# frgfm/Holocron

Hardware: AMD Instinct MI355X
Metric: images/sec fwd+bwd+AdaBelief, RepVGG-A0 bs256/GPU 224^2 (higher is better)
Workload: dtype bf16; 1 GPU; repvgg_a0 bf16 train step (fwd+bwd+AdaBelief), synthetic 224^2, bs=256 per MI355X (BASELINE.json configs[1]), random-init weights, 10 classes, CE label_smoothing 0.1; global_batch=256, parallelism=dp1, mode=weight gradients on a second stream; hipGraph replay of the full step, dump_outputs=/tmp/code/gt15__hip_graft__frgfm__Holocron/driver_out/dump_parent, deterministic=True

## Files before the change

### holocron_amd/_lib.py

```python
import ctypes as C
import os

import torch

_HERE = os.path.dirname(os.path.abspath(__file__))
LIB_PATH = os.environ.get("HC_LIB_PATH") or os.path.join(_HERE, "lib", "libholocron_hip.so")

HC_MAX_TAPS = 12
HC_MT_CHUNK = 8192
HC_STAT_REPLICAS = 128

c_void_p, c_int32, c_int64, c_float, c_double = C.c_void_p, C.c_int32, C.c_int64, C.c_float, C.c_double


class ConvClass(C.Structure):
    _fields_ = [("OHg", c_int32), ("OWg", c_int32), ("oy0", c_int32), ("ox0", c_int32), ("ostep", c_int32),
                ("istep", c_int32), ("ntaps", c_int32), ("tap", c_int32 * HC_MAX_TAPS)]


class ConvDesc(C.Structure):
    _fields_ = [("src0", c_void_p), ("src1", c_void_p), ("wpk", c_void_p), ("dst", c_void_p), ("resid", c_void_p),
                ("stats", c_void_p), ("bias", c_void_p), ("act", c_int32),
                ("N", c_int32), ("IH", c_int32), ("IW", c_int32), ("srcC", c_int32),
                ("OH", c_int32), ("OW", c_int32), ("Cout", c_int32), ("T", c_int32), ("nclass", c_int32),
# ... 162 lines not shown
    "hc_yolo1_loss_fwd": (c_int32, [c_void_p] * 3 + [c_int32] * 8 + [c_void_p] * 4 + [c_int32] + [c_void_p] * 4),
    "hc_yolo1_loss_bwd": (c_int32, [c_void_p] * 3 + [c_int32] * 8 + [c_void_p] * 4 + [c_int32] + [c_void_p] * 7),
    "hc_yolo1_decode": (c_int32, [c_void_p] * 3 + [c_int32] * 7 + [c_void_p] * 4),
    "hc_yolo_format_fwd": (c_int32, [c_void_p] * 2 + [c_int32] * 7 + [c_void_p] * 5),
    "hc_yolo_format_bwd": (c_int32, [c_void_p] * 3 + [c_int32] * 7 + [c_void_p] * 7),
    "hc_lamb_step": (c_int32, [c_void_p, c_int32, c_void_p, c_void_p, c_void_p, c_int32, c_void_p]),
    "hc_tadam_step": (c_int32, [c_void_p, c_int32, c_void_p, c_void_p, c_void_p, c_void_p, c_void_p, c_void_p, c_int32, c_void_p]),
    "hc_adan_step": (c_int32, [c_void_p, c_void_p, c_int32, c_void_p, c_void_p]),
    "hc_lookahead_sync": (c_int32, [c_void_p, c_int32, c_float, c_void_p]),
    "hc_multi_copy": (c_int32, [C.POINTER(MultiCopyDesc), c_void_p]),
    "hc_msbn_finalize": (c_int32, [C.POINTER(MsbnDesc), c_void_p]),
    "hc_msbn_bwd_finalize": (c_int32, [C.POINTER(MsbnDesc), c_void_p]),
    "hc_msbn_apply": (c_int32, [C.POINTER(MsbnIo), c_void_p, c_void_p, c_void_p, c_int32, c_void_p]),
    "hc_msbn_bwd_reduce": (c_int32, [C.POINTER(MsbnIo), c_void_p, c_int32, c_void_p, c_void_p, c_int32, c_void_p]),
    "hc_msbn_bwd_apply": (c_int32, [C.POINTER(MsbnIo), c_void_p, c_int32, c_void_p, c_void_p, c_int32, c_void_p]),
    "hc_dwrep_dgrad": (c_int32, [c_void_p, c_void_p, c_int32, c_void_p, c_void_p] + [c_int32] * 5 + [c_void_p]),
    "hc_conv_gather": (c_int32, [C.POINTER(ConvDesc), c_void_p]),
    "hc_conv_pointwise_supported": (c_int32, [C.POINTER(ConvDesc)]),
    "hc_conv_pointwise": (c_int32, [C.POINTER(ConvDesc), c_void_p]),
    "hc_conv_small": (c_int32, [C.POINTER(ConvSmallDesc), c_void_p]),
    "hc_conv_small_supported": (c_int32, [C.POINTER(ConvSmallDesc)]),
    "hc_conv_rows_fused_bwd_supported": (c_int32, [C.POINTER(ConvSmallDesc)]),
    "hc_conv_rows_fused_bwd": (c_int32, [C.POINTER(ConvSmallDesc), c_void_p, c_void_p, c_int32] + [c_void_p] * 8),
    "hc_conv_s2_supported": (c_int32, [C.POINTER(ConvS2Desc)]),
    "hc_conv_s2_fwd": (c_int32, [C.POINTER(ConvS2Desc), c_void_p]),
    "hc_conv_s2_dgrad_supported": (c_int32, [C.POINTER(ConvS2DgradDesc)]),
    "hc_conv_s2_dgrad": (c_int32, [C.POINTER(ConvS2DgradDesc), c_void_p]),
    "hc_conv_s2_stem_wgrad_ws_bytes": (c_int64, []),
    "hc_conv_s2_stem_wgrad": (c_int32, [c_void_p] * 6 + [c_int32] * 4 + [c_void_p]),
    "hc_conv_wgrad_ws_bytes": (c_int64, [C.POINTER(WgradDesc)]),
    "hc_conv_wgrad": (c_int32, [C.POINTER(WgradDesc), c_void_p]),
    "hc_conv_wgrad_group_supported": (c_int32, [C.POINTER(WgradGroupDesc)]),
    "hc_conv_wgrad_group_ws_bytes": (c_int64, [C.POINTER(WgradGroupDesc)]),
    "hc_conv_wgrad_group": (c_int32, [C.POINTER(WgradGroupDesc), c_void_p]),
    "hc_rep_wgrad_supported": (c_int32, [C.POINTER(RepWgradDesc)]),
    "hc_rep_wgrad_ws_bytes": (c_int64, [C.POINTER(RepWgradDesc)]),
    "hc_rep_wgrad_plan": (c_int32, [C.POINTER(RepWgradDesc), c_void_p]),
    "hc_rep_wgrad": (c_int32, [C.POINTER(RepWgradDesc), c_void_p]),
    "hc_pack_conv_weight": (c_int32, [c_void_p, c_void_p] + [c_int32] * 7 + [c_void_p]),
    "hc_pack_conv_weights_multi": (c_int32, [c_void_p, c_int32, c_int64, c_void_p]),
    "hc_nchw_to_nhwc_bf16": (c_int32, [c_void_p, c_void_p] + [c_int32] * 5 + [c_void_p]),
    "hc_nhwc_bf16_to_nchw": (c_int32, [c_void_p, c_void_p] + [c_int32] * 5 + [c_void_p]),
    "hc_im2col_small": (c_int32, [c_void_p, c_void_p] + [c_int32] * 11 + [c_void_p]),
    "hc_unpack_im2col_grad": (c_int32, [c_void_p, c_void_p] + [c_int32] * 6 + [c_void_p]),
    "hc_rep_bn_finalize": (c_int32, [C.POINTER(RepBnDesc), c_void_p]),
    "hc_rep_apply": (c_int32, [c_void_p] * 6 + [c_int64, c_int32, c_int32, c_void_p]),
# ... 152 lines not shown
```

### holocron_amd/csrc/conv_rows48.hip

```cpp
#include <type_traits>
#include "common.h"
#include "../../include/holocron_hip.h"

namespace crq {

constexpr int NT = 512, C = 48, CK = 2, PSC = C / 8 + 1, PS = PSC * 16, S3 = 9 * CK, S1 = CK, S = S3 + S1;
static_assert((PS / 8) % 4 == 2, "pixel pitch must be 2 x odd 8-byte units");

struct Args {
    hc_conv_small_desc d;
    int reps;
    int nunits;
    int delay;
};

template <int W>
struct Geo {
    static constexpr int RW = W > 64 ? 1 : 2;
    static constexpr int SEGW = (W + 15) / 16;
    static constexpr int NF = RW * SEGW;
    static constexpr int UR = 4 * RW;
    static constexpr int WW = W + 1;
    static constexpr int NSLOT = (UR + 2) * WW + 1;
    static constexpr int NDMA = (NSLOT * PS + 1023) / 1024;
    static constexpr int WIN = NDMA * 1024;
    static constexpr int SMEM = 2 * WIN + 64 + 1024;
    static_assert(SMEM <= 160 * 1024, "LDS budget");
};

__device__ __forceinline__ u32x4 uniform_rsrc(const void* p, unsigned bytes) {
    const unsigned long long v = reinterpret_cast<unsigned long long>(p);
    u32x4 r;
    r[0] = __builtin_amdgcn_readfirstlane((unsigned)v);
    r[1] = __builtin_amdgcn_readfirstlane((unsigned)(v >> 32) & 0xffffu);
    r[2] = __builtin_amdgcn_readfirstlane(bytes);
    r[3] = 0x00020000u;
    return r;
}
__device__ __forceinline__ bf16x8 frag2(const char* lo_p, const char* hi_p) {
    const u32x2 lo = *reinterpret_cast<const u32x2*>(lo_p), hi = *reinterpret_cast<const u32x2*>(hi_p);
    const u32x4 v = {lo[0], lo[1], hi[0], hi[1]};
    return __builtin_bit_cast(bf16x8, v);
}
__device__ __forceinline__ float row16_sum(float v) {
    v += __builtin_bit_cast(float, __builtin_amdgcn_update_dpp(0, __builtin_bit_cast(int, v), 0x128, 0xf, 0xf, false));
    v += __builtin_bit_cast(float, __builtin_amdgcn_update_dpp(0, __builtin_bit_cast(int, v), 0x124, 0xf, 0xf, false));
    v += __builtin_bit_cast(float, __builtin_amdgcn_update_dpp(0, __builtin_bit_cast(int, v), 0x122, 0xf, 0xf, false));
    v += __builtin_bit_cast(float, __builtin_amdgcn_update_dpp(0, __builtin_bit_cast(int, v), 0x121, 0xf, 0xf, false));
    return v;
}

template <int W, int MODE, int DBG>
__global__ __launch_bounds__(NT, 1) void conv_rows48_kernel(const Args a) {
    using G = Geo<W>;
    constexpr int WW = G::WW, NF = G::NF, UR = G::UR, RW = G::RW, SEGW = G::SEGW;
    extern __shared__ __attribute__((aligned(1024))) char smem[];
    const hc_conv_small_desc& d = a.d;
    const int tid = threadIdx.x, lane = tid & 63;
    const int wid = __builtin_amdgcn_readfirstlane(tid >> 6);
    const int team = wid >> 2, pw = wid & 3;
    const int H = d.H, UPI = H / UR;
    const unsigned lds0 = hc_lds_addr(smem);
    const int px = lane & 15, g = lane >> 4;
    const int region = team * G::WIN;
    int* cnt = reinterpret_cast<int*>(smem + 2 * G::WIN) + team * 8;
    int gen = 0;

    if (tid < 16) reinterpret_cast<int*>(smem + 2 * G::WIN)[tid] = 0;
    __syncthreads();

    auto team_sync = [&]() __attribute__((always_inline)) {
        asm volatile("s_waitcnt vmcnt(0) lgkmcnt(0)" ::: "memory");
        gen += 4;
        if (lane == 0) __hip_atomic_fetch_add(cnt, 1, __ATOMIC_RELAXED, __HIP_MEMORY_SCOPE_WORKGROUP);
        while (__hip_atomic_load(cnt, __ATOMIC_RELAXED, __HIP_MEMORY_SCOPE_WORKGROUP) < gen) __builtin_amdgcn_s_sleep(1);
        asm volatile("" ::: "memory");
    };

    const unsigned act_bytes = (unsigned)d.N * H * W * C * 2u;
    const u32x4 rsA = uniform_rsrc(d.srcA, act_bytes);
    const u32x4 rsB = uniform_rsrc(MODE == 1 ? d.srcB : d.srcA, act_bytes);
    const __amdgpu_buffer_rsrc_t rsw = make_rsrc(d.w3, (unsigned)(S * C * 64));

    const unsigned wl = (unsigned)((lane & 15) * 64 + g * 16);
    u32x4 af[3][3];
    auto load_a = [&](int buf, int s) __attribute__((always_inline)) {
        if (DBG & 4) return;
#pragma unroll
        for (int f = 0; f < 3; ++f) af[buf][f] = buf_load16(rsw, wl, (unsigned)(s * (C * 64) + f * 1024));
    };

    auto stage_window = [&](const u32x4 rs, int n, int row0, int j0, int j1) __attribute__((always_inline)) {
        if (DBG & 8) return;
        const unsigned img = (unsigned)n * (unsigned)(H * W * C * 2);
        for (int j = j0 + pw; j < j1; j += 4) {
            const int J = j * 64 + lane;
            const int slot = J / PSC, c = J - slot * PSC;
            const int r = slot / WW, x = slot - r * WW;
            const int ih = row0 - 1 + r;
            const bool ok = c < PSC - 1 && slot < G::NSLOT && x >= 1 && ih >= 0 && ih < H;
            const unsigned off = img + (unsigned)((ih * W + x - 1) * C * 2 + c * 16);
            hc_dma16(rs, lds0 + (unsigned)(region + j * 1024), ok ? off : HC_OOB);
        }
    };

    const int vb = region + ((pw * RW + 1) * WW + px + 1) * PS + g * 8;
    bf16x8 bfr[2][NF];
    auto load_b = [&](int buf, int bofs, int second) __attribute__((always_inline)) {
        if (DBG & 2) return;
        const char* sb = smem + vb + bofs;
#pragma unroll
        for (int i = 0; i < NF; ++i) {
            const int o = ((i / SEGW) * WW + 16 * (i % SEGW)) * PS;
            bfr[buf][i] = frag2(sb + o, sb + o + second);
        }
    };

    f32x4 acc[3][NF];
    auto zero_acc = [&]() __attribute__((always_inline)) {
#pragma unroll
        for (int f = 0; f < 3; ++f)
#pragma unroll
            for (int i = 0; i < NF; ++i) acc[f][i] = f32x4{0.f, 0.f, 0.f, 0.f};
    };
    auto mfma_step = [&](int ab, int bb) __attribute__((always_inline)) {
#pragma unroll
        for (int i = 0; i < NF; ++i)
#pragma unroll
            for (int f = 0; f < 3; ++f) {
                if (DBG & 1) acc[f][i][0] += __builtin_bit_cast(float, af[ab][f][0]) * (float)bfr[bb][i][0];
                else acc[f][i] = __builtin_amdgcn_mfma_f32_16x16x32_bf16(__builtin_bit_cast(bf16x8, af[ab][f]), bfr[bb][i], acc[f][i], 0, 0, 0);
            }
    };
    auto step = [&](int a3, int par, int s, int bnext, int second_next, bool prefetch) __attribute__((always_inline)) {
        if (s + 2 < S) load_a((a3 + 2) % 3, s + 2);
        if (prefetch) load_b(par ^ 1, bnext, second_next);
        __builtin_amdgcn_sched_barrier(0);
        mfma_step(a3, par);
        __builtin_amdgcn_sched_barrier(0);
    };

    const int cbase = 8 * g;
    auto epilogue = [&](void* outp, float* stats, const void* residp, int n, int row0) __attribute__((always_inline)) {
        if (DBG & 16) {
            float t = 0.f;
#pragma unroll
            for (int f = 0; f < 3; ++f)
#pragma unroll
                for (int i = 0; i < NF; ++i) t += acc[f][i][0];
            if (t == 123.456f) reinterpret_cast<float*>(outp)[tid] = t;
            return;
        }
        const size_t img = (size_t)n * H * W * C;
        __builtin_amdgcn_sched_barrier(0);
        float st[2][12];
#pragma unroll
        for (int k = 0; k < 2; ++k)
#pragma unroll
            for (int e = 0; e < 12; ++e) st[k][e] = 0.f;
#pragma unroll
        for (int i = 0; i < NF; ++i) {
            const int row = row0 + pw * RW + i / SEGW, col = 16 * (i % SEGW) + px;
            const bool ok = col < W;
            const size_t e0 = img + (size_t)(row * W + (ok ? col : 0)) * C + cbase;
            bf16_t* op = reinterpret_cast<bf16_t*>(outp) + e0;
            const bf16_t* rp = residp != nullptr ? reinterpret_cast<const bf16_t*>(residp) + e0 : nullptr;
            u32x4 r16 = {0u, 0u, 0u, 0u};
            u32x2 r8 = {0u, 0u};
            if (rp != nullptr && ok) {
                r16 = *reinterpret_cast<const u32x4*>(rp);
                r8 = *reinterpret_cast<const u32x2*>(rp + 32 - 4 * g);
            }
            u32x2 pk[3];
#pragma unroll
            for (int f = 0; f < 3; ++f) {
                f32x4 v = acc[f][i];
                if (stats != nullptr) {
#pragma unroll
                    for (int e = 0; e < 4; ++e) {
                        const float x = ok ? v[e] : 0.f;
                        st[0][f * 4 + e] += x;
                        st[1][f * 4 + e] += x * x;
                    }
                }
                const unsigned ra = f == 0 ? r16[0] : (f == 1 ? r16[2] : r8[0]), rb = f == 0 ? r16[1] : (f == 1 ? r16[3] : r8[1]);
                v[0] += bf16lo(ra); v[1] += bf16hi(ra); v[2] += bf16lo(rb); v[3] += bf16hi(rb);
                pk[f] = u32x2{pack_bf16x2(v[0], v[1]), pack_bf16x2(v[2], v[3])};
            }
            if (ok) {
                *reinterpret_cast<u32x4*>(op) = u32x4{pk[0][0], pk[0][1], pk[1][0], pk[1][1]};
                *reinterpret_cast<u32x2*>(op + 32 - 4 * g) = pk[2];
            }
        }
        if (stats != nullptr) {
            float* rep = stats + (size_t)((blockIdx.x * 8 + wid) % a.reps) * 2 * C + cbase;
#pragma unroll
            for (int k = 0; k < 2; ++k) {
                float mine = 0.f;
#pragma unroll
                for (int e = 0; e < 12; ++e) {
                    const float x = row16_sum(st[k][e]);
                    mine = px == e ? x : mine;
                }
                if (px < 12) atomicAdd(rep + k * C + (px < 8 ? px : 24 - 4 * g + px), mine);
            }
        }
    };

    if (team == 1)
        for (int i = 0; i < a.delay; ++i) __builtin_amdgcn_s_sleep(64);
    bool first = true;
    for (int u = 2 * blockIdx.x + team; u < a.nunits; u += 2 * gridDim.x) {
        const int n = u / UPI, row0 = (u - n * UPI) * UR;
        if (!first) team_sync();
        first = false;
        stage_window(rsA, n, row0, 0, G::NDMA);
        load_a(0, 0);
        load_a(1, 1);
        team_sync();
        zero_acc();
        load_b(0, (-WW - 1) * PS, 32);
#pragma nounroll
        for (int kh = 0; kh < 3; ++kh) {
            const int rofs = (kh - 1) * WW * PS;
#pragma unroll
            for (int t = 0; t < 6; ++t) {
                const int kw = t >> 1, kk = t & 1;
                int bnext, second;
                bool pf = true;
                if (kk == 0) { bnext = rofs + (kw - 1) * PS + 64; second = 0; }
                else if (t < 5) { bnext = rofs + kw * PS; second = 32; }
                else {
                    bnext = kh < 2 ? kh * WW * PS - PS : 0;
                    second = 32;
                    pf = kh < 2 || MODE == 0;
                }
                step(t % 3, kk, 6 * kh + t, bnext, second, pf);
            }
        }
        if (MODE == 0) {
            epilogue(d.out3, d.stats3, nullptr, n, row0);
            zero_acc();
        } else {
            team_sync();
            stage_window(rsB, n, row0, (WW * PS) / 1024, ((UR + 1) * WW * PS + PS + 1023) / 1024);
            team_sync();
            load_b(0, 0, 32);
        }
        step(0, 0, S3, 64, 0, true);
        step(1, 1, S3 + 1, 0, 0, false);
        if (MODE == 0) epilogue(d.out1, d.stats1, nullptr, n, row0);
        else epilogue(d.out3, nullptr, d.resid, n, row0);
    }
}

template <int W>
bool shape_ok(const hc_conv_small_desc& d) {
    return d.C == C && d.Cout == C && d.W == W && d.H >= Geo<W>::UR && d.H % Geo<W>::UR == 0 && d.N >= 1 &&
           (double)d.N * d.H * d.W * C * 2.0 < 2147483000.0;
}

template <int W, int MODE, int DBG>
void launch1(const Args& a, hipStream_t st) {
    auto kern = conv_rows48_kernel<W, MODE, DBG>;
    constexpr int smem = Geo<W>::SMEM;
    static bool attr_set = false;
    if (!attr_set) {
        (void)hipFuncSetAttribute(reinterpret_cast<const void*>(kern), hipFuncAttributeMaxDynamicSharedMemorySize, smem);
        attr_set = true;
    }
    int grid = (a.nunits + 1) / 2;
    if (grid > 256) grid = 256;
    hipLaunchKernelGGL(kern, dim3(grid), dim3(NT), smem, st, a);
}

template <int W>
void launch(Args& a, hipStream_t st) {
    static const int dbg = getenv("HC_CRQ_DBG") ? atoi(getenv("HC_CRQ_DBG")) : 0;
    constexpr int delay = 2;
    a.nunits = a.d.N * (a.d.H / Geo<W>::UR);
    a.delay = delay;
    const bool dg = (a.d.mode & 1) == 1;
#define CRQ_CASE(k) case k: if (dg) launch1<W, 1, k>(a, st); else launch1<W, 0, k>(a, st); break;
    switch (dbg) {
        CRQ_CASE(1) CRQ_CASE(2) CRQ_CASE(4) CRQ_CASE(7) CRQ_CASE(8) CRQ_CASE(16) CRQ_CASE(24) CRQ_CASE(31)
        default: if (dg) launch1<W, 1, 0>(a, st); else launch1<W, 0, 0>(a, st); break;
    }
#undef CRQ_CASE
}

}

bool hc_conv_rows48_supported(const hc_conv_small_desc& d) {
    static const int on = [] { const char* e = getenv("HC_CONV_ROWS48"); return e == nullptr ? 1 : atoi(e); }();
    if (on <= 0 || (d.mode & HC_CONV_SMALL_ROWS_IMAGE) == 0 || (d.mode & ~(HC_CONV_SMALL_ROWS_IMAGE | 1)) != 0) return false;
    if ((d.mode & 1) && on < 2) return false;
    return crq::shape_ok<112>(d) || crq::shape_ok<56>(d);
}
int hc_conv_rows48_launch(const hc_conv_small_desc& d, hipStream_t st) {
    if (!hc_conv_rows48_supported(d)) return HC_ERR_ARG;
    const bool dg = (d.mode & 1) == 1;
    if (d.srcA == nullptr || d.w3 == nullptr || d.out3 == nullptr) return HC_ERR_ARG;
    if (!dg && d.out1 == nullptr) return HC_ERR_ARG;
    if (dg && d.srcB == nullptr) return HC_ERR_ARG;
    if (!dg && (d.stats3 == nullptr) != (d.stats1 == nullptr)) return HC_ERR_ARG;
    crq::Args a;
    a.d = d;
    a.reps = hc_get_stat_replicas();
    if (d.W == 112) crq::launch<112>(a, st);
    else crq::launch<56>(a, st);
    return hc_launch_status();
}
```

### holocron_amd/nn/repblock_op.py

```python
import ctypes as C

import os

import torch

from .. import _lib
from .._lib import ConvS2Desc, ConvS2DgradDesc, PackItem, RepBnBwdDesc, RepBnDesc, StemBwdDesc, StemDesc, check, ptr, stream
from ..ops import conv as cv

STEM_KPAD = 32
FUSED_BWD = os.environ.get("HC_REP_FUSED_BWD", "1") != "0"


class ZeroPool:

    def __init__(self):
        self.buf = None
        self.used = 0
        self.high = 0
        self.depth = 0
        self.gen = 0
        self.retired = []
        self.graph_users = 0
        self.buf_captured = False

    def _retire(self):
        if self.buf is not None and self.buf_captured:
            self.retired.append(self.buf)
        self.buf, self.buf_captured = None, False

    def release_retired(self):
        self.graph_users = max(0, self.graph_users - 1)
        if self.graph_users == 0:
            self.retired = []
# ... 85 lines not shown
class RepState:

    def __init__(self, stride, identity):
        self.stride = stride
        self.identity = identity
        self.emit_stats = False
        self.fwd_cache = cv.PackCache()
        self.bwd_cache = cv.PackCache()
        self.desc = {}
        self.bn = None
        self.eps = 1e-5
        self.momentum = 0.1
        self.training = True
        self.last_out_stats = None
        self.packed = None
        self.packed_key = None
        self.pack_table = {}
        self.rows_image = (False, False)
        self.stack_fwd = False
        self.s2 = False
        self.s2_images = None
        self.s2_dgrad = False
        self.s2_dimg = None

    @staticmethod
    def weights_key(w3, w1):
        return (w3.data_ptr(), w3._version, w1.data_ptr(), w1._version, cv.weights_epoch())

    def pack_items(self, w3, w1):
        Cout, Cin = w3.shape[0], w3.shape[1]
        dev = w3.device
        stem = (Cin % 16) != 0
        if self.s2:
            return self._pack_items_s2(w3, w1, Cout, Cin, dev, stem)
        self.stack_fwd = (stem or (self.stride == 2 and Cin <= 48)) and Cout % 4 == 0
        if self.packed is None or self.packed[0].device != dev:
            if self.stack_fwd:
                self.packed = (torch.zeros((2 * Cout, 1, STEM_KPAD) if stem else (2 * Cout, 9, Cin), dtype=torch.bfloat16, device=dev),
                               None, None if stem else torch.empty((Cin, 10, Cout), dtype=torch.bfloat16, device=dev))
            elif any(self.rows_image):
                rf, rb = self.rows_image
                self.packed = (cv.rows_image(Cout, dev) if rf else torch.empty((Cout, 9, Cin), dtype=torch.bfloat16, device=dev),
                               None if rf else torch.empty((Cout, 1, Cin), dtype=torch.bfloat16, device=dev),
                               cv.rows_image(Cout, dev) if rb else torch.empty((Cin, 10, Cout), dtype=torch.bfloat16, device=dev))
            elif stem:
                self.packed = (torch.zeros((Cout, 1, STEM_KPAD), dtype=torch.bfloat16, device=dev),
                               torch.zeros((Cout, 1, STEM_KPAD), dtype=torch.bfloat16, device=dev), None)
            else:
                self.packed = (torch.empty((Cout, 9, Cin), dtype=torch.bfloat16, device=dev),
                               torch.empty((Cout, 1, Cin), dtype=torch.bfloat16, device=dev),
                               torch.empty((Cin, 10, Cout), dtype=torch.bfloat16, device=dev))
            self.packed_key = None
        wp3, wp1, wpd = self.packed
        if self.stack_fwd:
            if stem:
                return [(w3, wp3, Cout, Cin, 3, 3, 2, 0, STEM_KPAD), (w1, wp3[Cout:], Cout, Cin, 1, 1, 2, 4 * Cin, STEM_KPAD)]
            return [(w3, wp3, Cout, Cin, 3, 3, 0, 0, 9), (w1, wp3[Cout:], Cout, Cin, 1, 1, 0, 4, 9),
                    (w3, wpd, Cout, Cin, 3, 3, 1, 0, 10), (w1, wpd, Cout, Cin, 1, 1, 1, 9, 10)]
        if any(self.rows_image):
            rf, rb = self.rows_image
            fwd = ([(w3, wp3, Cout, Cin, 3, 3, 3, 0, 10), (w1, wp3, Cout, Cin, 1, 1, 3, 9, 10)] if rf else
                   [(w3, wp3, Cout, Cin, 3, 3, 0, 0, 9), (w1, wp1, Cout, Cin, 1, 1, 0, 0, 1)])
            bwd = ([(w3, wpd, Cout, Cin, 3, 3, 4, 0, 10), (w1, wpd, Cout, Cin, 1, 1, 4, 9, 10)] if rb else
                   [(w3, wpd, Cout, Cin, 3, 3, 1, 0, 10), (w1, wpd, Cout, Cin, 1, 1, 1, 9, 10)])
            return fwd + bwd
        if stem:
            return [(w3, wp3, Cout, Cin, 3, 3, 2, 0, STEM_KPAD), (w1, wp1, Cout, Cin, 1, 1, 2, 4 * Cin, STEM_KPAD)]
        return [(w3, wp3, Cout, Cin, 3, 3, 0, 0, 9), (w1, wp1, Cout, Cin, 1, 1, 0, 0, 1),
                (w3, wpd, Cout, Cin, 3, 3, 1, 0, 10), (w1, wpd, Cout, Cin, 1, 1, 1, 9, 10)]

    def _pack_items_s2(self, w3, w1, Cout, Cin, dev, stem):
        if stem:
            s3, s1, s1b, mode, tap1 = 2, 1, 0, 6, 4
        else:
            pt = Cin // 8
# ... 53 lines not shown
                dg = None
            sf = sd = None
            rows = (False, False)
            if Cin % 16 == 0 and s == 1:
                sf = cv.conv_small_desc(N, H, W, Cin, Cout, cv.ROWS_IMAGE)
                sd = cv.conv_small_desc(N, H, W, Cout, Cin, cv.ROWS_IMAGE | 1)
                rows = (sf is not None, sd is not None)
                if sf is None:
                    sf = cv.conv_small_desc(N, H, W, Cin, Cout, 0)
                if sd is None:
                    sd = cv.conv_small_desc(N, H, W, Cout, Cin, 1)
            s2d = None
            if s == 2:
                c = ConvS2Desc()
                c.N, c.H, c.W, c.Cin, c.Cout, c.x_nchw_f32 = N, H, W, Cin, Cout, 1 if Cin % 16 else 0
                if _lib.load().hc_conv_s2_supported(C.byref(c)):
                    s2d = c
            s2g = None
            if s == 2 and s2d is not None and Cin % 16 == 0:
                c = ConvS2DgradDesc()
                c.N, c.H, c.W, c.Cin, c.Cout = N, H, W, Cin, Cout
                if _lib.load().hc_conv_s2_dgrad_supported(C.byref(c)):
                    s2g = c
            self.desc[key] = (f3, f1, dg, sf, sd, rows, s2d, s2g)
        rows = self.desc[key][5]
        s2, s2g = self.desc[key][6] is not None, self.desc[key][7] is not None
        if rows != self.rows_image or s2 != self.s2 or s2g != self.s2_dgrad:
            self.rows_image, self.s2, self.s2_dgrad, self.packed, self.packed_key = rows, s2, s2g, None, None
        return self.desc[key][:5]

    def s2_desc(self, N, Cin, H, W, Cout):
        self.descs(N, Cin, H, W, Cout)
        return self.desc[(N, Cin, H, W, Cout)][6]


def _stats_of(x):
    st = getattr(x, "_hc_stats", None)
    if st is not None:
        return st
    N, Cc, H, W = x.shape
    st = POOL.take((_lib.stat_replicas(), 2, Cc), x.device)
    with cv.profiled("bn_elementwise", 0.0, N * H * W * Cc * 2.0):
        check(_lib.load().hc_channel_stats(ptr(x), ptr(st), N * H * W, Cc, stream()), "hc_channel_stats")
    return st


def block_convs_forward(st, src, w3, w1, geom, stats=None, stem_cin=None):
    N, Cin, H, W, Cout = geom
    f3, f1, _, sf, _ = st.descs(N, Cin, H, W, Cout)
    OH, OW = f3.OH, f3.OW
    dev = src.device
# ... 47 lines not shown
        cv.launch_conv_small_dgrad(sdg, dy3, dy1, wpd, dx, resid=dxid)
    else:
        cv.launch_conv(dg, dy3, wpd, dx, src1=dy1, resid=dxid)
    return dx


def fused_dgrad_desc(st, geom):
    N, Cin, H, W, Cout = geom
    sdg = st.descs(N, Cin, H, W, Cout)[4]
    if sdg is None or not st.rows_image[1] or Cin != Cout or not _lib.load().hc_conv_rows_fused_bwd_supported(C.byref(sdg)):
        return None
    return sdg


def block_dgrad_fused(st, sdg, g, coef, act, y3, y1, x, bcoef, w3, w1, bufs=None):
    wpd = st.ensure_packed(w3, w1)[2]
    dy3, dy1, dxid, dx = bufs if bufs is not None else (torch.empty_like(y3), torch.empty_like(y1), torch.empty_like(x), torch.empty_like(x))
    sdg.srcA, sdg.srcB, sdg.resid, sdg.w3, sdg.w1, sdg.out3, sdg.out1, sdg.stats3, sdg.stats1 = None, None, None, ptr(wpd), None, ptr(dx), None, None, None
    tb = x.numel() * 2.0
    with cv.profiled("conv_rows", 2.0 * sdg.N * sdg.H * sdg.W * sdg.Cout * 10 * sdg.C, 8 * tb):
        check(_lib.load().hc_conv_rows_fused_bwd(C.byref(sdg), ptr(g), ptr(coef), act, ptr(y3), ptr(y1), ptr(x), ptr(bcoef), ptr(dy3),
                                                 ptr(dy1), ptr(dxid), stream()), "hc_conv_rows_fused_bwd")
    return dy3, dy1, dxid, dx


def block_wgrad(st, src, dy3, dy1, w3, w1, geom, stem_cin=None, defer=False):
    N, Cin, H, W, Cout = geom
    lib = _lib.load()
    npix = dy3.shape[0] * dy3.shape[2] * dy3.shape[3]
    if stem_cin is not None and src.dtype == torch.float32:
        dw3 = torch.empty_like(w3, dtype=torch.float32)
        dw1 = torch.empty_like(w1, dtype=torch.float32)
        ws = torch.empty((int(lib.hc_conv_s2_stem_wgrad_ws_bytes()),), dtype=torch.uint8, device=src.device)
        with cv.profiled("conv_wgrad", 2.0 * npix * Cout * 10 * stem_cin, src.numel() * 4.0 + 2 * dy3.numel() * 2.0):
            rc = lib.hc_conv_s2_stem_wgrad(ptr(src), ptr(dy3), ptr(dy1), ptr(dw3), ptr(dw1), ptr(ws), N, H, W, 0, stream())
        if rc == 0:
            return dw3, dw1
        src = cv.im2col_small(src, 3, 3, st.stride, 1, STEM_KPAD)
    if stem_cin is not None:
        K = STEM_KPAD
        dwc3 = cv.conv_wgrad(src, dy3, K, Cout, 1, 1, 1, 0, flops=2.0 * npix * Cout * 9 * stem_cin)
        dwc1 = cv.conv_wgrad(src, dy1, K, Cout, 1, 1, 1, 0, flops=2.0 * npix * Cout * stem_cin)
        dw3 = torch.empty_like(w3, dtype=torch.float32)
        check(lib.hc_unpack_im2col_grad(ptr(dwc3), ptr(dw3), Cout, stem_cin, 3, 3, K, 0, stream()), "hc_unpack_im2col_grad")
        dw1 = dwc1.view(Cout, K)[:, 4 * stem_cin:5 * stem_cin].reshape(Cout, stem_cin, 1, 1).contiguous()
        return dw3, dw1
# ... 136 lines not shown
        ctx.red = None
        with cv.profiled("bn_elementwise", 0.0, tb * (4 if st.identity else 3)):
            check(lib.hc_rep_bwd_reduce_z(ptr(g), ptr(coef), act, ptr(y3), ptr(y1), ptr(xid), ptr(red), npix, Cout, stream()),
                  "hc_rep_bwd_reduce_z")
        nb = 3 if st.identity else 2
        dgam = torch.empty((3, Cout), dtype=torch.float32, device=dev)
        dbet = torch.empty((3, Cout), dtype=torch.float32, device=dev)
        bcoef = torch.empty((9, Cout), dtype=torch.float32, device=dev)
        d = RepBnBwdDesc()
        d.red, d.save, d.bcoef = ptr(red), ptr(save), ptr(bcoef)
        gam = (g3, g1, g0)
        for b in range(3):
            live = b < nb
            d.gamma[b] = ptr(gam[b]) if live else None
            d.dgamma[b] = ptr(dgam[b]) if live else None
            d.dbeta[b] = ptr(dbet[b]) if live else None
        d.C, d.count, d.has_identity, d.accumulate = Cout, npix, 1 if st.identity else 0, 0
        d.frozen = 0 if ctx.was_training else 1
        with cv.profiled("bn_finalize", 0.0, 0.0):
            check(lib.hc_rep_bn_bwd_finalize(C.byref(d), stream()), "hc_rep_bn_bwd_finalize")

        dx = None
        geom = (N, Cin, H, W, Cout)
        fdg = fused_dgrad_desc(st, geom) if (FUSED_BWD and st.identity and ctx.needs_input_grad[0] and not ctx.stem) else None
        if fdg is not None:
            dy3, dy1, dxid, dx = block_dgrad_fused(st, fdg, g, coef, act, y3, y1, src, bcoef, w3, w1)
        else:
            dy3 = torch.empty_like(y3)
            dy1 = torch.empty_like(y1)
            dxid = torch.empty_like(src) if st.identity else None
            with cv.profiled("bn_elementwise", 0.0, tb * (7 if st.identity else 5)):
                check(lib.hc_rep_bwd_apply_z(ptr(g), ptr(coef), act, ptr(y3), ptr(y1), ptr(xid), ptr(bcoef), ptr(dy3), ptr(dy1),
                                             ptr(dxid), npix, Cout, stream()), "hc_rep_bwd_apply_z")
            if ctx.needs_input_grad[0]:
                if ctx.stem:
                    raise NotImplementedError("input gradient of the im2col stem path")
                dx = block_dgrad(st, dy3, dy1, dxid, w3, w1, geom)

        with cv.side_stream_for_wgrad((w3, w1), (src, dy3, dy1)) as side:
            dw3, dw1 = block_wgrad(st, src, dy3, dy1, w3, w1, geom, Cin if ctx.stem else None, defer=True)
            side.produced(dw3, dw1)
        return (dx, dw3, dw1, dgam[0], dbet[0], dgam[1], dbet[1],
                dgam[2] if st.identity else None, dbet[2] if st.identity else None, None, None)


def rep_block_forward(x, w3, w1, bn3, bn1, bn0, st, relu=True):
    st.bn = [(bn3.running_mean, bn3.running_var, bn3.num_batches_tracked),
             (bn1.running_mean, bn1.running_var, bn1.num_batches_tracked),
             (bn0.running_mean, bn0.running_var, bn0.num_batches_tracked) if bn0 is not None else (None, None, None)]
# ... 13 lines not shown
```

### include/holocron_hip.h

```cpp
#ifndef HOLOCRON_HIP_H
#define HOLOCRON_HIP_H
#include <stdint.h>
#ifdef __cplusplus
extern "C" {
#endif

typedef void* hc_stream_t;

#define HC_MAX_TAPS 12
#define HC_STAT_REPLICAS 128
#define HC_STAT_REPLICAS_DETERMINISTIC 32768
int hc_set_deterministic(int on);
int hc_get_deterministic(void);
int hc_get_stat_replicas(void);

typedef struct {
    int32_t OHg, OWg, oy0, ox0, ostep, istep, ntaps;
    int32_t tap[HC_MAX_TAPS];
} hc_conv_class;
#define HC_TAP(dy, dx, src, wt) \
    ((int32_t)(((uint32_t)(dy) & 0xffu) | (((uint32_t)(dx) & 0xffu) << 8) | ((uint32_t)(src) << 16) | ((uint32_t)(wt) << 24)))

typedef struct {
    const void* src0;
// ... 23 lines not shown
int hc_conv_gather(const hc_conv_desc* d, hc_stream_t stream);
int hc_conv_pointwise_supported(const hc_conv_desc* d);
int hc_conv_pointwise(const hc_conv_desc* d, hc_stream_t stream);

#define HC_CONV_SMALL_ROWS_IMAGE 4
typedef struct {
    const void* srcA;
    const void* srcB;
    const void* w3;
    const void* w1;
    void* out3;
    void* out1;
    const void* resid;
    float* stats3;
    float* stats1;
    int32_t w3_rstride, w1_rstride;
    int32_t N, H, W, C, Cout, mode;
} hc_conv_small_desc;
int hc_conv_small(const hc_conv_small_desc* d, hc_stream_t stream);
int hc_conv_small_supported(const hc_conv_small_desc* d);
int hc_conv_rows_fused_bwd_supported(const hc_conv_small_desc* d);
int hc_conv_rows_fused_bwd(const hc_conv_small_desc* d, const void* g, const float* coef, int32_t act, const void* y3, const void* y1,
                           const void* x, const float* bcoef, void* dy3, void* dy1, void* dxid, hc_stream_t stream);

typedef struct {
    const void* x;
    const void* w3img;
    const void* w1img;
    void* y3;
    void* y1;
    float* stats3;
    float* stats1;
    int32_t N, H, W, Cin, Cout, x_nchw_f32;
} hc_conv_s2_desc;
int hc_conv_s2_supported(const hc_conv_s2_desc* d);
int hc_conv_s2_fwd(const hc_conv_s2_desc* d, hc_stream_t stream);
typedef struct {
    const void* dy3;
    const void* dy1;
    const void* wimg;
    void* dx;
    int32_t N, H, W, Cin, Cout;
} hc_conv_s2_dgrad_desc;
int hc_conv_s2_dgrad_supported(const hc_conv_s2_dgrad_desc* d);
int hc_conv_s2_dgrad(const hc_conv_s2_dgrad_desc* d, hc_stream_t stream);
int64_t hc_conv_s2_stem_wgrad_ws_bytes(void);
// ... 452 lines not shown
```

Before: 26590 images/sec.

## Fuse RepVGG BN-backward elementwise into the 48-channel rows dgrad kernel

Adds a third kernel mode to the 48-channel row-tiled conv kernel. In this mode each team walks a strip of row units per image and, in a prologue, computes the rep-block backward elementwise step (dz, then dy3/dy1/dxid) straight into the LDS window. It writes those gradients to global memory only for owned rows and reuses halo rows already computed by the previous unit. This removes a separate elementwise kernel and the global round-trip of dy3 before dgrad, at the cost of more register pressure, halo recompute at strip edges and a more complex prologue. It is enabled by default for identity blocks at width 112 and 56 when the existing fused path does not apply.

```diff
diff --git a/holocron_amd/_lib.py b/holocron_amd/_lib.py
--- a/holocron_amd/_lib.py
+++ b/holocron_amd/_lib.py
@@ -208,6 +208,9 @@
     "hc_conv_small_supported": (c_int32, [C.POINTER(ConvSmallDesc)]),
     "hc_conv_rows_fused_bwd_supported": (c_int32, [C.POINTER(ConvSmallDesc)]),
     "hc_conv_rows_fused_bwd": (c_int32, [C.POINTER(ConvSmallDesc), c_void_p, c_void_p, c_int32] + [c_void_p] * 8),
+    "hc_conv_rows48_fused_bwd_supported": (c_int32, [C.POINTER(ConvSmallDesc)]),
+    "hc_conv_rows48_fused_bwd": (c_int32, [C.POINTER(ConvSmallDesc), c_void_p, c_void_p, c_int32] + [c_void_p] * 7 + [c_int32, c_void_p]),
+    "hc_conv_rows48_dgrad": (c_int32, [C.POINTER(ConvSmallDesc), c_void_p]),
     "hc_conv_s2_supported": (c_int32, [C.POINTER(ConvS2Desc)]),
     "hc_conv_s2_fwd": (c_int32, [C.POINTER(ConvS2Desc), c_void_p]),
     "hc_conv_s2_dgrad_supported": (c_int32, [C.POINTER(ConvS2DgradDesc)]),
diff --git a/holocron_amd/csrc/conv_rows48.hip b/holocron_amd/csrc/conv_rows48.hip
--- a/holocron_amd/csrc/conv_rows48.hip
+++ b/holocron_amd/csrc/conv_rows48.hip
@@ -1,5 +1,6 @@
 #include <type_traits>
 #include "common.h"
+#include "rep_ew.h"
 #include "../../include/holocron_hip.h"
 
 namespace crq {
@@ -12,6 +13,14 @@
     int reps;
     int nunits;
     int delay;
+};
+struct FusedArgs : Args {
+    const void *g, *y3, *y1, *x;
+    const float *coef, *bcoef;
+    void* dy3;
+    int act;
+    int spi;
+    int nstrips;
 };
 
 template <int W>
@@ -37,6 +46,9 @@
     r[3] = 0x00020000u;
     return r;
 }
+__device__ __forceinline__ void dma16_sc1(const u32x4 rsrc, unsigned lds_off, unsigned voff) {
+    asm volatile("s_mov_b32 m0, %0\n\ts_nop 0\n\tbuffer_load_dwordx4 %1, %2, 0 offen sc1 lds" ::"s"(lds_off), "v"(voff), "s"(rsrc) : "memory");
+}
 __device__ __forceinline__ bf16x8 frag2(const char* lo_p, const char* hi_p) {
     const u32x2 lo = *reinterpret_cast<const u32x2*>(lo_p), hi = *reinterpret_cast<const u32x2*>(hi_p);
     const u32x4 v = {lo[0], lo[1], hi[0], hi[1]};
@@ -51,17 +63,18 @@
 }
 
 template <int W, int MODE, int DBG>
-__global__ __launch_bounds__(NT, 1) void conv_rows48_kernel(const Args a) {
+__global__ __launch_bounds__(NT, 1) void conv_rows48_kernel(const std::conditional_t<MODE == 2, FusedArgs, Args> a) {
     using G = Geo<W>;
     constexpr int WW = G::WW, NF = G::NF, UR = G::UR, RW = G::RW, SEGW = G::SEGW;
     extern __shared__ __attribute__((aligned(1024))) char smem[];
     const hc_conv_small_desc& d = a.d;
-    const int tid = threadIdx.x, lane = tid & 63;
+    const int tid = threadIdx.x;
+    int lane = tid & 63;
     const int wid = __builtin_amdgcn_readfirstlane(tid >> 6);
     const int team = wid >> 2, pw = wid & 3;
     const int H = d.H, UPI = H / UR;
     const unsigned lds0 = hc_lds_addr(smem);
-    const int px = lane & 15, g = lane >> 4;
+    int px = lane & 15, g = lane >> 4;
     const int region = team * G::WIN;
     int* cnt = reinterpret_cast<int*>(smem + 2 * G::WIN) + team * 8;
     int gen = 0;
@@ -79,7 +92,7 @@
 
     const unsigned act_bytes = (unsigned)d.N * H * W * C * 2u;
     const u32x4 rsA = uniform_rsrc(d.srcA, act_bytes);
-    const u32x4 rsB = uniform_rsrc(MODE == 1 ? d.srcB : d.srcA, act_bytes);
+    const u32x4 rsB = uniform_rsrc(MODE != 0 ? d.srcB : d.srcA, act_bytes);
     const __amdgpu_buffer_rsrc_t rsw = make_rsrc(d.w3, (unsigned)(S * C * 64));
 
     const unsigned wl = (unsigned)((lane & 15) * 64 + g * 16);
@@ -100,11 +113,119 @@
             const int ih = row0 - 1 + r;
             const bool ok = c < PSC - 1 && slot < G::NSLOT && x >= 1 && ih >= 0 && ih < H;
             const unsigned off = img + (unsigned)((ih * W + x - 1) * C * 2 + c * 16);
-            hc_dma16(rs, lds0 + (unsigned)(region + j * 1024), ok ? off : HC_OOB);
-        }
-    };
-
-    const int vb = region + ((pw * RW + 1) * WW + px + 1) * PS + g * 8;
+            if (MODE == 2) dma16_sc1(rs, lds0 + (unsigned)(region + j * 1024), ok ? off : HC_OOB);
+            else hc_dma16(rs, lds0 + (unsigned)(region + j * 1024), ok ? off : HC_OOB);
+        }
+    };
+
+    auto fused_prologue = [&](int n, int row0, bool fresh, int own0, int own1) __attribute__((always_inline)) {
+        if constexpr (MODE == 2) {
+            if (DBG & 32) return;
+            constexpr int CG = C / 8, PPS = 256 / CG, BATCH = 2, NFB = (2 * W + PPS - 1) / PPS;
+            int tt = pw * 64 + lane;
+            asm volatile("" : "+v"(tt));
+            const int pl = tt / CG, chunk = tt - pl * CG;
+            const bool active = pl < PPS;
+            const int HW = H * W, NP = (UR + 2) * W;
+            const int gp0 = (row0 - 1) * W;
+            const __amdgpu_buffer_rsrc_t rg = make_rsrc(a.g, act_bytes), r3 = make_rsrc(a.y3, act_bytes), r1 = make_rsrc(a.y1, act_bytes),
+                                         rx = make_rsrc(a.x, act_bytes), rd3 = make_rsrc(a.dy3, act_bytes),
+                                         rd1 = make_rsrc(d.srcB, act_bytes), rd0 = make_rsrc(d.resid, act_bytes);
+            u32x4 fb[NFB];
+            if (!fresh) {
+#pragma unroll
+                for (int k = 0; k < NFB; ++k) {
+                    const int p = pl + k * PPS;
+                    const unsigned off = active && p < 2 * W ? (unsigned)(((n * HW + gp0 + p) * CG + chunk) * 16) : HC_OOB;
+                    fb[k] = __builtin_amdgcn_raw_buffer_load_b128(rd3, off, 0, 16);
+                }
+            }
+            __builtin_amdgcn_sched_barrier(0);
+            for (int j = pw; j < G::NDMA; j += 4) {
+                const int J = j * 64 + lane;
+                const int slot = J / PSC, c = J - slot * PSC;
+                const int r = slot / WW, x = slot - r * WW;
+                const int ih = row0 - 1 + r;
+                const bool ok = c < PSC - 1 && slot < G::NSLOT && x >= 1 && ih >= 0 && ih < H;
+                if (!ok) *reinterpret_cast<u32x4*>(smem + region + J * 16) = u32x4{0u, 0u, 0u, 0u};
+            }
+            if (!fresh) {
+#pragma unroll
+                for (int k = 0; k < NFB; ++k) {
+                    const int p = pl + k * PPS;
+                    if (active && p < 2 * W) {
+                        const int r = p / W, x = p - r * W;
+                        *reinterpret_cast<u32x4*>(smem + region + (r * WW + x + 1) * PS + chunk * 16) = fb[k];
+                    }
+                }
+            }
+            __builtin_amdgcn_sched_barrier(0);
+            int c0 = chunk * 8;
+            asm volatile("" : "+v"(c0));
+            float a3[8], a1[8], a0[8], sh[8], A3[8], B3[8], C3[8], A1[8], B1[8], C1[8], A0[8], B0[8], C0[8];
+            load8f(a.coef + c0, a3); load8f(a.coef + C + c0, a1); load8f(a.coef + 2 * C + c0, a0); load8f(a.coef + 3 * C + c0, sh);
+            load8f(a.bcoef + 0 * C + c0, A3); load8f(a.bcoef + 1 * C + c0, B3); load8f(a.bcoef + 2 * C + c0, C3);
+            load8f(a.bcoef + 3 * C + c0, A1); load8f(a.bcoef + 4 * C + c0, B1); load8f(a.bcoef + 5 * C + c0, C1);
+            load8f(a.bcoef + 6 * C + c0, A0); load8f(a.bcoef + 7 * C + c0, B0); load8f(a.bcoef + 8 * C + c0, C0);
+            const int act = a.act;
+            const int so0 = own0 * W, so1 = own1 * W;
+            struct Batch { u32x4 vg[BATCH], v3[BATCH], v1[BATCH], vx[BATCH]; unsigned off[BATCH]; };
+            auto request = [&](Batch& q, int pb) __attribute__((always_inline)) {
+#pragma unroll
+                for (int b = 0; b < BATCH; ++b) {
+                    const int p = pb + b * PPS, gp = gp0 + p;
+                    const bool ok = active && p < NP && gp >= 0 && gp < HW;
+                    q.off[b] = ok ? (unsigned)(((n * HW + gp) * CG + chunk) * 16) : HC_OOB;
+                    q.vg[b] = buf_load16(rg, q.off[b]);
+                    q.v3[b] = buf_load16(r3, q.off[b]);
+                    q.v1[b] = buf_load16(r1, q.off[b]);
+                    q.vx[b] = buf_load16(rx, q.off[b]);
+                }
+            };
+            auto finish = [&](const Batch& q, int pb) __attribute__((always_inline)) {
+#pragma unroll
+                for (int b = 0; b < BATCH; ++b) {
+                    const int p = pb + b * PPS, gp = gp0 + p;
+                    float fg[8], f3[8], f1[8], f0[8], o3[8], o1[8], o0[8];
+                    unpack8(q.vg[b], fg); unpack8(q.v3[b], f3); unpack8(q.v1[b], f1); unpack8(q.vx[b], f0);
+#pragma unroll
+                    for (int i = 0; i < 8; ++i) {
+                        const float fo = act == 1 ? rep_preact<true>(a3[i], f3[i], a1[i], f1[i], a0[i], f0[i], sh[i]) : 1.f;
+                        const float dz = rep_bwd_dz(fo, fg[i]);
+                        o3[i] = rep_bwd_branch(A3[i], dz, B3[i], f3[i], C3[i]);
+                        o1[i] = rep_bwd_branch(A1[i], dz, B1[i], f1[i], C1[i]);
+                        o0[i] = rep_bwd_branch(A0[i], dz, B0[i], f0[i], C0[i]);
+                    }
+                    const u32x4 p3 = pack8(o3);
+                    if (q.off[b] != HC_OOB) {
+                        const int r = p / W, x = p - r * W;
+                        *reinterpret_cast<u32x4*>(smem + region + (r * WW + x + 1) * PS + chunk * 16) = p3;
+                    }
+                    const unsigned so = (gp >= so0 && gp < so1) ? q.off[b] : HC_OOB;
+                    __builtin_amdgcn_raw_buffer_store_b128(p3, rd3, so, 0, 0);
+                    __builtin_amdgcn_raw_buffer_store_b128(pack8(o1), rd1, so, 0, 0);
+                    __builtin_amdgcn_raw_buffer_store_b128(pack8(o0), rd0, so, 0, 0);
+                }
+            };
+            constexpr int STEP = BATCH * PPS;
+            const int pstart = (fresh ? 0 : 2 * W) + pl;
+            Batch q0, q1;
+            request(q0, pstart);
+#pragma nounroll
+            for (int pb = pstart; pb < NP + pl; pb += 2 * STEP) {
+                request(q1, pb + STEP);
+                __builtin_amdgcn_sched_barrier(0);
+                finish(q0, pb);
+                __builtin_amdgcn_sched_barrier(0);
+                request(q0, pb + 2 * STEP);
+                __builtin_amdgcn_sched_barrier(0);
+                finish(q1, pb + STEP);
+                __builtin_amdgcn_sched_barrier(0);
+            }
+        }
+    };
+
+    int vb = region + ((pw * RW + 1) * WW + px + 1) * PS + g * 8;
     bf16x8 bfr[2][NF];
     auto load_b = [&](int buf, int bofs, int second) __attribute__((always_inline)) {
         if (DBG & 2) return;
@@ -140,8 +261,9 @@
         __builtin_amdgcn_sched_barrier(0);
     };
 
-    const int cbase = 8 * g;
+    const int cbase0 = 8 * g;
     auto epilogue = [&](void* outp, float* stats, const void* residp, int n, int row0) __attribute__((always_inline)) {
+        const int cbase = MODE == 2 ? 8 * g : cbase0;
         if (DBG & 16) {
             float t = 0.f;
 #pragma unroll
@@ -168,8 +290,14 @@
             u32x4 r16 = {0u, 0u, 0u, 0u};
             u32x2 r8 = {0u, 0u};
             if (rp != nullptr && ok) {
-                r16 = *reinterpret_cast<const u32x4*>(rp);
-                r8 = *reinterpret_cast<const u32x2*>(rp + 32 - 4 * g);
+                if constexpr (MODE == 2) {
+                    const __amdgpu_buffer_rsrc_t rr = make_rsrc(residp, act_bytes);
+                    r16 = __builtin_amdgcn_raw_buffer_load_b128(rr, (unsigned)e0 * 2u, 0, 16);
+                    r8 = __builtin_amdgcn_raw_buffer_load_b64(rr, (unsigned)e0 * 2u + (unsigned)(64 - 8 * g), 0, 16);
+                } else {
+                    r16 = *reinterpret_cast<const u32x4*>(rp);
+                    r8 = *reinterpret_cast<const u32x2*>(rp + 32 - 4 * g);
+                }
             }
             u32x2 pk[3];
 #pragma unroll
@@ -207,17 +335,7 @@
         }
     };
 
-    if (team == 1)
-        for (int i = 0; i < a.delay; ++i) __builtin_amdgcn_s_sleep(64);
-    bool first = true;
-    for (int u = 2 * blockIdx.x + team; u < a.nunits; u += 2 * gridDim.x) {
-        const int n = u / UPI, row0 = (u - n * UPI) * UR;
-        if (!first) team_sync();
-        first = false;
-        stage_window(rsA, n, row0, 0, G::NDMA);
-        load_a(0, 0);
-        load_a(1, 1);
-        team_sync();
+    auto unit_tail = [&](int n, int row0) __attribute__((always_inline)) {
         zero_acc();
         load_b(0, (-WW - 1) * PS, 32);
 #pragma nounroll
@@ -251,6 +369,42 @@
         step(1, 1, S3 + 1, 0, 0, false);
         if (MODE == 0) epilogue(d.out1, d.stats1, nullptr, n, row0);
         else epilogue(d.out3, nullptr, d.resid, n, row0);
+    };
+
+    if (team == 1)
+        for (int i = 0; i < a.delay; ++i) __builtin_amdgcn_s_sleep(64);
+    bool first = true;
+    if constexpr (MODE == 2) {
+        const int spi = a.spi, base = UPI / spi, rem = UPI - base * spi;
+        for (int s = 2 * blockIdx.x + team; s < a.nstrips; s += 2 * gridDim.x) {
+            const int n = s / spi, k = s - n * spi;
+            const int u0 = k * base + (k < rem ? k : rem), L = base + (k < rem ? 1 : 0);
+            const int own0 = u0 * UR, own1 = (u0 + L) * UR;
+            for (int j = 0; j < L; ++j) {
+                const int row0 = own0 + j * UR;
+                if (!first) team_sync();
+                first = false;
+                asm volatile("" : "+v"(lane));
+                fused_prologue(n, row0, j == 0, own0, own1);
+                load_a(0, 0);
+                load_a(1, 1);
+                team_sync();
+                asm volatile("" : "+v"(px), "+v"(g));
+                vb = region + ((pw * RW + 1) * WW + px + 1) * PS + g * 8;
+                unit_tail(n, row0);
+            }
+        }
+    } else {
+        for (int u = 2 * blockIdx.x + team; u < a.nunits; u += 2 * gridDim.x) {
+            const int n = u / UPI, row0 = (u - n * UPI) * UR;
+            if (!first) team_sync();
+            first = false;
+            stage_window(rsA, n, row0, 0, G::NDMA);
+            load_a(0, 0);
+            load_a(1, 1);
+            team_sync();
+            unit_tail(n, row0);
+        }
     }
 }
 
@@ -261,7 +415,7 @@
 }
 
 template <int W, int MODE, int DBG>
-void launch1(const Args& a, hipStream_t st) {
+void launch1(const std::conditional_t<MODE == 2, FusedArgs, Args>& a, hipStream_t st) {
     auto kern = conv_rows48_kernel<W, MODE, DBG>;
     constexpr int smem = Geo<W>::SMEM;
     static bool attr_set = false;
@@ -269,18 +423,20 @@
         (void)hipFuncSetAttribute(reinterpret_cast<const void*>(kern), hipFuncAttributeMaxDynamicSharedMemorySize, smem);
         attr_set = true;
     }
-    int grid = (a.nunits + 1) / 2;
+    int work = a.nunits;
+    if constexpr (MODE == 2) work = a.nstrips;
+    int grid = (work + 1) / 2;
     if (grid > 256) grid = 256;
     hipLaunchKernelGGL(kern, dim3(grid), dim3(NT), smem, st, a);
 }
 
+constexpr int DELAY = 2;
+
 template <int W>
-void launch(Args& a, hipStream_t st) {
+void launch(Args& a, bool dg, hipStream_t st) {
     static const int dbg = getenv("HC_CRQ_DBG") ? atoi(getenv("HC_CRQ_DBG")) : 0;
-    constexpr int delay = 2;
     a.nunits = a.d.N * (a.d.H / Geo<W>::UR);
-    a.delay = delay;
-    const bool dg = (a.d.mode & 1) == 1;
+    a.delay = DELAY;
 #define CRQ_CASE(k) case k: if (dg) launch1<W, 1, k>(a, st); else launch1<W, 0, k>(a, st); break;
     switch (dbg) {
         CRQ_CASE(1) CRQ_CASE(2) CRQ_CASE(4) CRQ_CASE(7) CRQ_CASE(8) CRQ_CASE(16) CRQ_CASE(24) CRQ_CASE(31)
@@ -289,16 +445,37 @@
 #undef CRQ_CASE
 }
 
-}
-
+template <int W>
+void launch_fused(FusedArgs& a, int strip_units, hipStream_t st) {
+    static const int dbg = getenv("HC_CRQ_DBG") ? atoi(getenv("HC_CRQ_DBG")) : 0;
+    const int upi = a.d.H / Geo<W>::UR;
+    int spi = strip_units > 0 ? (upi + strip_units - 1) / strip_units : (512 + a.d.N - 1) / a.d.N;
+    if (spi > upi) spi = upi;
+    a.nunits = a.d.N * upi;
+    a.spi = spi;
+    a.nstrips = a.d.N * spi;
+    a.delay = DELAY;
+#define CRQ_CASE(k) case k: launch1<W, 2, k>(a, st); break;
+    switch (dbg) {
+        CRQ_CASE(1) CRQ_CASE(2) CRQ_CASE(4) CRQ_CASE(8) CRQ_CASE(16) CRQ_CASE(31) CRQ_CASE(32)
+        default: launch1<W, 2, 0>(a, st); break;
+    }
+#undef CRQ_CASE
+}
+
+}
+
+static int rows48_switch() {
+    static const int on = [] { const char* e = getenv("HC_CONV_ROWS48"); return e == nullptr ? 1 : atoi(e); }();
+    return on;
+}
 bool hc_conv_rows48_supported(const hc_conv_small_desc& d) {
-    static const int on = [] { const char* e = getenv("HC_CONV_ROWS48"); return e == nullptr ? 1 : atoi(e); }();
+    const int on = rows48_switch();
     if (on <= 0 || (d.mode & HC_CONV_SMALL_ROWS_IMAGE) == 0 || (d.mode & ~(HC_CONV_SMALL_ROWS_IMAGE | 1)) != 0) return false;
     if ((d.mode & 1) && on < 2) return false;
     return crq::shape_ok<112>(d) || crq::shape_ok<56>(d);
 }
-int hc_conv_rows48_launch(const hc_conv_small_desc& d, hipStream_t st) {
-    if (!hc_conv_rows48_supported(d)) return HC_ERR_ARG;
+static int rows48_launch(const hc_conv_small_desc& d, hipStream_t st) {
     const bool dg = (d.mode & 1) == 1;
     if (d.srcA == nullptr || d.w3 == nullptr || d.out3 == nullptr) return HC_ERR_ARG;
     if (!dg && d.out1 == nullptr) return HC_ERR_ARG;
@@ -307,7 +484,39 @@
     crq::Args a;
     a.d = d;
     a.reps = hc_get_stat_replicas();
-    if (d.W == 112) crq::launch<112>(a, st);
-    else crq::launch<56>(a, st);
+    if (d.W == 112) crq::launch<112>(a, dg, st);
+    else crq::launch<56>(a, dg, st);
     return hc_launch_status();
 }
+int hc_conv_rows48_launch(const hc_conv_small_desc& d, hipStream_t st) {
+    if (!hc_conv_rows48_supported(d)) return HC_ERR_ARG;
+    return rows48_launch(d, st);
+}
+
+extern "C" int hc_conv_rows48_dgrad(const hc_conv_small_desc* dp, hc_stream_t stream) {
+    if (dp == nullptr || dp->mode != (HC_CONV_SMALL_ROWS_IMAGE | 1) || !(crq::shape_ok<112>(*dp) || crq::shape_ok<56>(*dp))) return HC_ERR_ARG;
+    return rows48_launch(*dp, (hipStream_t)stream);
+}
+
+extern "C" int hc_conv_rows48_fused_bwd_supported(const hc_conv_small_desc* dp) {
+    return dp != nullptr && rows48_switch() > 0 && dp->mode == (HC_CONV_SMALL_ROWS_IMAGE | 1) &&
+                   (crq::shape_ok<112>(*dp) || crq::shape_ok<56>(*dp)) ? 1 : 0;
+}
+extern "C" int hc_conv_rows48_fused_bwd(const hc_conv_small_desc* dp, const void* g, const float* coef, int32_t act, const void* y3,
+                                        const void* y1, const void* x, const float* bcoef, void* dy3, void* dy1, void* dxid,
+                                        int32_t strip_units, hc_stream_t stream) {
+    if (!hc_conv_rows48_fused_bwd_supported(dp)) return HC_ERR_ARG;
+    if (dp->w3 == nullptr || dp->out3 == nullptr || g == nullptr || coef == nullptr || y3 == nullptr || y1 == nullptr || x == nullptr ||
+        bcoef == nullptr || dy3 == nullptr || dy1 == nullptr || dxid == nullptr || (act != 0 && act != 1) || strip_units < 0)
+        return HC_ERR_ARG;
+    crq::FusedArgs a;
+    a.d = *dp;
+    a.d.srcA = dy3;
+    a.d.srcB = dy1;
+    a.d.resid = dxid;
+    a.reps = hc_get_stat_replicas();
+    a.g = g; a.y3 = y3; a.y1 = y1; a.x = x; a.coef = coef; a.bcoef = bcoef; a.dy3 = dy3; a.act = act;
+    if (dp->W == 112) crq::launch_fused<112>(a, strip_units, (hipStream_t)stream);
+    else crq::launch_fused<56>(a, strip_units, (hipStream_t)stream);
+    return hc_launch_status();
+}
diff --git a/holocron_amd/nn/repblock_op.py b/holocron_amd/nn/repblock_op.py
--- a/holocron_amd/nn/repblock_op.py
+++ b/holocron_amd/nn/repblock_op.py
@@ -10,6 +10,8 @@
 
 STEM_KPAD = 32
 FUSED_BWD = os.environ.get("HC_REP_FUSED_BWD", "1") != "0"
+FUSED_BWD48 = os.environ.get("HC_REP_FUSED_BWD48", "1") != "0"
+FUSED_BWD48_WIDTHS = (112, 56)
 
 
 class ZeroPool:
@@ -141,6 +143,8 @@
         self.s2_images = None
         self.s2_dgrad = False
         self.s2_dimg = None
+        self.fused48 = False
+        self.dimg48 = None
 
     @staticmethod
     def weights_key(w3, w1):
@@ -170,6 +174,16 @@
                                torch.empty((Cout, 1, Cin), dtype=torch.bfloat16, device=dev),
                                torch.empty((Cin, 10, Cout), dtype=torch.bfloat16, device=dev))
             self.packed_key = None
+        wp3, wp1, wpd = self.packed
+        if self.fused48:
+            if self.dimg48 is None or self.dimg48.device != dev:
+                self.dimg48 = cv.rows_image(Cout, dev)
+                self.packed_key = None
+            return self._pack_items_plain(w3, w1, Cout, Cin, stem) + [(w3, self.dimg48, Cout, Cin, 3, 3, 4, 0, 10),
+                                                                    (w1, self.dimg48, Cout, Cin, 1, 1, 4, 9, 10)]
+        return self._pack_items_plain(w3, w1, Cout, Cin, stem)
+
+    def _pack_items_plain(self, w3, w1, Cout, Cin, stem):
         wp3, wp1, wpd = self.packed
         if self.stack_fwd:
             if stem:
@@ -269,11 +283,17 @@
                 c.N, c.H, c.W, c.Cin, c.Cout = N, H, W, Cin, Cout
                 if _lib.load().hc_conv_s2_dgrad_supported(C.byref(c)):
                     s2g = c
-            self.desc[key] = (f3, f1, dg, sf, sd, rows, s2d, s2g)
+            f48 = None
+            if self.identity and s == 1 and Cin == Cout:
+                c = _lib.ConvSmallDesc()
+                c.N, c.H, c.W, c.C, c.Cout, c.mode = N, H, W, Cout, Cin, cv.ROWS_IMAGE | 1
+                if _lib.load().hc_conv_rows48_fused_bwd_supported(C.byref(c)):
+                    f48 = c
+            self.desc[key] = (f3, f1, dg, sf, sd, rows, s2d, s2g, f48)
         rows = self.desc[key][5]
-        s2, s2g = self.desc[key][6] is not None, self.desc[key][7] is not None
-        if rows != self.rows_image or s2 != self.s2 or s2g != self.s2_dgrad:
-            self.rows_image, self.s2, self.s2_dgrad, self.packed, self.packed_key = rows, s2, s2g, None, None
+        s2, s2g, f48 = self.desc[key][6] is not None, self.desc[key][7] is not None, self.desc[key][8] is not None
+        if rows != self.rows_image or s2 != self.s2 or s2g != self.s2_dgrad or f48 != self.fused48:
+            self.rows_image, self.s2, self.s2_dgrad, self.fused48, self.packed, self.packed_key = rows, s2, s2g, f48, None, None
         return self.desc[key][:5]
 
     def s2_desc(self, N, Cin, H, W, Cout):
@@ -367,6 +387,34 @@
         check(_lib.load().hc_conv_rows_fused_bwd(C.byref(sdg), ptr(g), ptr(coef), act, ptr(y3), ptr(y1), ptr(x), ptr(bcoef), ptr(dy3),
                                                  ptr(dy1), ptr(dxid), stream()), "hc_conv_rows_fused_bwd")
     return dy3, dy1, dxid, dx
+
+
+def fused48_dgrad_desc(st, geom):
+    N, Cin, H, W, Cout = geom
+    st.descs(N, Cin, H, W, Cout)
+    return st.desc[(N, Cin, H, W, Cout)][8]
+
+
+def block_dgrad_fused48(st, sdg, g, coef, act, y3, y1, x, bcoef, w3, w1, bufs=None, strip_units=0):
+    st.ensure_packed(w3, w1)
+    dy3, dy1, dxid, dx = bufs if bufs is not None else (torch.empty_like(y3), torch.empty_like(y1), torch.empty_like(x), torch.empty_like(x))
+    sdg.srcA, sdg.srcB, sdg.resid, sdg.w3, sdg.w1, sdg.out3, sdg.out1, sdg.stats3, sdg.stats1 = None, None, None, ptr(st.dimg48), None, ptr(dx), None, None, None
+    tb = x.numel() * 2.0
+    with cv.profiled("conv_rows", 2.0 * sdg.N * sdg.H * sdg.W * sdg.Cout * 10 * sdg.C, 8 * tb):
+        check(_lib.load().hc_conv_rows48_fused_bwd(C.byref(sdg), ptr(g), ptr(coef), act, ptr(y3), ptr(y1), ptr(x), ptr(bcoef), ptr(dy3),
+                                                   ptr(dy1), ptr(dxid), strip_units, stream()), "hc_conv_rows48_fused_bwd")
+    return dy3, dy1, dxid, dx
+
+
+def block_dgrad_rows48(st, dy3, dy1, dxid, w3, w1, geom):
+    sdg = fused48_dgrad_desc(st, geom)
+    if sdg is None:
+        raise _lib.HipError("hc_conv_rows48_dgrad does not take %r" % (geom,))
+    st.ensure_packed(w3, w1)
+    dx = torch.empty_like(dxid)
+    sdg.srcA, sdg.srcB, sdg.resid, sdg.w3, sdg.w1, sdg.out3, sdg.out1, sdg.stats3, sdg.stats1 = ptr(dy3), ptr(dy1), ptr(dxid), ptr(st.dimg48), None, ptr(dx), None, None, None
+    check(_lib.load().hc_conv_rows48_dgrad(C.byref(sdg), stream()), "hc_conv_rows48_dgrad")
+    return dx
 
 
 def block_wgrad(st, src, dy3, dy1, w3, w1, geom, stem_cin=None, defer=False):
@@ -549,9 +597,13 @@
 
         dx = None
         geom = (N, Cin, H, W, Cout)
-        fdg = fused_dgrad_desc(st, geom) if (FUSED_BWD and st.identity and ctx.needs_input_grad[0] and not ctx.stem) else None
+        fuse = FUSED_BWD and st.identity and ctx.needs_input_grad[0] and not ctx.stem
+        fdg = fused_dgrad_desc(st, geom) if fuse else None
+        f48 = fused48_dgrad_desc(st, geom) if (fuse and fdg is None and FUSED_BWD48 and W in FUSED_BWD48_WIDTHS) else None
         if fdg is not None:
             dy3, dy1, dxid, dx = block_dgrad_fused(st, fdg, g, coef, act, y3, y1, src, bcoef, w3, w1)
+        elif f48 is not None:
+            dy3, dy1, dxid, dx = block_dgrad_fused48(st, f48, g, coef, act, y3, y1, src, bcoef, w3, w1)
         else:
             dy3 = torch.empty_like(y3)
             dy1 = torch.empty_like(y1)
diff --git a/include/holocron_hip.h b/include/holocron_hip.h
--- a/include/holocron_hip.h
+++ b/include/holocron_hip.h
@@ -69,6 +69,10 @@
 int hc_conv_rows_fused_bwd_supported(const hc_conv_small_desc* d);
 int hc_conv_rows_fused_bwd(const hc_conv_small_desc* d, const void* g, const float* coef, int32_t act, const void* y3, const void* y1,
                            const void* x, const float* bcoef, void* dy3, void* dy1, void* dxid, hc_stream_t stream);
+int hc_conv_rows48_fused_bwd_supported(const hc_conv_small_desc* d);
+int hc_conv_rows48_fused_bwd(const hc_conv_small_desc* d, const void* g, const float* coef, int32_t act, const void* y3, const void* y1,
+                             const void* x, const float* bcoef, void* dy3, void* dy1, void* dxid, int32_t strip_units, hc_stream_t stream);
+int hc_conv_rows48_dgrad(const hc_conv_small_desc* d, hc_stream_t stream);
 
 typedef struct {
     const void* x;
```

Result: no change. 26820 images/sec (median of 6 runs) (+0.9%).
